# norlab-ulaval/norlab_icp_mapper

Measured on AMD Instinct MI355X. Metric: ICP iterations/sec, 100k-pt scan vs 1M-pt map, higher is better.
Workload: dtype f32; 1 GPU; single synthetic 100000-pt scan vs 1000000-pt map, point-to-point ICP, KDTreeMatcher knn 1 maxDist 2.0 epsilon 0, TrimmedDist 0.85, fixed 20 iterations per registration; chain=p2p, scene=box+pillars sigma=0.01 seeds 42/43/44 (SURVEY.md 8d), parallelism=scan-sharded x1, map replicated

## Files before the change

### norlab_icp_mapper_amd/csrc/common.h

```cpp
#pragma once

#include <hip/hip_runtime.h>
#include <stdint.h>
#include <math.h>
#include <cstring>
#include <string>
#include <vector>
#include <unordered_map>
#include <mutex>
#include <map>
#include <cstdlib>
#include <shared_mutex>

#include "../../include/icpmi.h"

#define ICPMI_NV 32
#define ICPMI_MAX_OUTLIER 8
#define ICPMI_MAX_SMOOTH 16
#define ICPMI_SEL_BINS 2048
#ifndef ICPMI_S2_COPIES
#define ICPMI_S2_COPIES 8
#endif
#define ICPMI_S2_C0 4096
#define ICPMI_S2_F0 (ICPMI_S2_C0 + ICPMI_S2_COPIES * 256)
// ... 127 lines not shown
    double hrot[ICPMI_MAX_SMOOTH + 1];
    double htr[ICPMI_MAX_SMOOTH + 1];
    double init_q[4];
    unsigned sel_prefix;
    unsigned sel_rank;
    unsigned n_valid;
    unsigned sel_prefix_l[3];
    unsigned sel_rank_l[3];
    float limits[ICPMI_MAX_OUTLIER];
    unsigned vt_valid;
    float vt_ratio;
    float robust_med;
    float robust_scale;
    long long pairs;
    double wsum;
    unsigned hard_count;
    unsigned ticket;
    unsigned long long hard_total;
    unsigned seq;
    unsigned long long dbg[24];
    float T_prev[16];
    float T_out[16];
    unsigned long long t_start, t_done;
    unsigned long long t_nn_begin, t_nn_sum;
    unsigned nn_count, pad_nn;
};

#ifdef __HIPCC__
__device__ __forceinline__ void nn_stamp_open(IcpState* st) { st->t_nn_begin = (unsigned long long)wall_clock64(); }
__device__ __forceinline__ void nn_stamp_close(IcpState* st)
{
    const unsigned long long b = st->t_nn_begin;
    if (b) { st->t_nn_sum += (unsigned long long)wall_clock64() - b; ++st->nn_count; st->t_nn_begin = 0; }
}
#endif


inline std::shared_mutex& capture_gate() { static std::shared_mutex* m = new std::shared_mutex; return *m; }
struct CaptureGate {
    CaptureGate() { capture_gate().lock_shared(); }
    ~CaptureGate() { capture_gate().unlock_shared(); }
    CaptureGate(const CaptureGate&) = delete;
    CaptureGate& operator=(const CaptureGate&) = delete;
};

struct LoopGraph {
    hipGraphExec_t exec = nullptr; uint64_t sig = 0; int uses = 0; bool sorted = false;
    int len = 0; unsigned long used = 0;
    bool holds(uint64_t s) const { return exec && sig == s; }
    void reset() { if (exec) hipGraphExecDestroy(exec); *this = LoopGraph(); }
};
struct LoopGraphs {
    LoopGraph fixed, batch, seg[2], heads[4];
    unsigned long clock = 0;
    void reset() { fixed.reset(); batch.reset(); for (LoopGraph& g : seg) g.reset(); for (LoopGraph& g : heads) g.reset(); }
};

struct DevBlockCache {
    struct Live { size_t bytes; int dev; };
    std::mutex mu;
    std::unordered_map<void*, Live> live;
    std::map<int, std::multimap<size_t, void*>> idle_of;
    size_t idle_bytes = 0, limit = 0;
    long handles = 0;
    bool on = true;
    DevBlockCache()
// ... 374 lines not shown
        HIP_TRY(c, hipStreamSynchronize(c->stream));
        return ICPMI_OK;
    }
    HIP_TRY(c, hipMemcpyAsync(c->h_pin, src0, b0, hipMemcpyDeviceToHost, c->stream));
    if (b1) HIP_TRY(c, hipMemcpyAsync(c->h_pin + b0, src1, b1, hipMemcpyDeviceToHost, c->stream));
    HIP_TRY(c, hipStreamSynchronize(c->stream));
    memcpy(dst0, c->h_pin, b0);
    if (b1) memcpy(dst1, c->h_pin + b0, b1);
    return ICPMI_OK;
}
static inline icpmi_status read_back(icpmi_ctx* c, void* dst, const void* src, size_t bytes) { return read_back2(c, dst, src, bytes, nullptr, nullptr, 0); }

#define ICPMI_UP_SLOT 1024
#define ICPMI_UP_SLOTS 64
static inline icpmi_status upload_small(icpmi_ctx* c, void* d_dst, const void* h_src, size_t bytes)
{
    if (!c->h_pin || bytes > ICPMI_UP_SLOT) {
        HIP_TRY(c, hipMemcpyAsync(d_dst, h_src, bytes, hipMemcpyHostToDevice, c->stream));
        return ICPMI_OK;
    }
    unsigned char* slot = c->h_pin + ICPMI_PIN_BYTES + (size_t)(c->up_next++ % ICPMI_UP_SLOTS) * ICPMI_UP_SLOT;
    memcpy(slot, h_src, bytes);
    HIP_TRY(c, hipMemcpyAsync(d_dst, slot, bytes, hipMemcpyHostToDevice, c->stream));
    return ICPMI_OK;
}

template <typename T>
static inline T* scratch_get(icpmi_ctx* c, int k, size_t count)
{
    if (c->scratch[k].ensure(c, (count ? count : 1) * sizeof(T)) != ICPMI_OK) { c->last_error = "out of device memory (operator scratch)"; return nullptr; }
    return (T*)c->scratch[k].get();
}

__device__ __forceinline__ float3 xf_point(const float* __restrict__ T, float x, float y, float z, float w)
{
    float3 o;
    o.x = fmaf(T[12], w, fmaf(T[8], z, fmaf(T[4], y, T[0] * x)));
    o.y = fmaf(T[13], w, fmaf(T[9], z, fmaf(T[5], y, T[1] * x)));
    o.z = fmaf(T[14], w, fmaf(T[10], z, fmaf(T[6], y, T[2] * x)));
    return o;
}

__device__ __forceinline__ float sqdist3(float ax, float ay, float az, float bx, float by, float bz)
{
    const float dx = ax - bx, dy = ay - by, dz = az - bz;
    return fmaf(dz, dz, fmaf(dy, dy, dx * dx));
}

__device__ __forceinline__ unsigned long long pack_key(float d2, unsigned id)
{
    return ((unsigned long long)__float_as_uint(d2) << 32) | (unsigned long long)id;
}

__device__ __forceinline__ float sqrt_up(float x) { return __builtin_amdgcn_sqrtf(x) * 1.0000005f; }

__device__ __forceinline__ unsigned fmix32(unsigned h)
{
    h ^= h >> 16; h *= 0x85ebca6bu; h ^= h >> 13; h *= 0xc2b2ae35u; h ^= h >> 16;
    return h;
}

__device__ __forceinline__ unsigned long long mix64(unsigned long long x)
{
    x ^= x >> 33; x *= 0xff51afd7ed558ccdull; x ^= x >> 33; x *= 0xc4ceb9fe1a85ec53ull; x ^= x >> 33;
    return x;
}
// ... 290 lines not shown
```

### norlab_icp_mapper_amd/csrc/loop.hip

```cpp
#include "common.h"
#include "solve.h"
#include <cstring>

namespace {

template <int PASS, int MODE = 0>
__global__ __launch_bounds__(256) void sel_hist_kernel(const float* __restrict__ d2, int64_t count,
                                                       const IcpState* __restrict__ st, unsigned* __restrict__ ghist, int nb_scale = 0)
{
    if (st->done) return;
    if (blockIdx.x == 0 && threadIdx.x == 0) nn_stamp_close(const_cast<IcpState*>(st));
    if (MODE != 0 && nb_scale != 0 && st->iter + 1 > nb_scale) return;
    if (MODE == 3 && st->iter != 0) return;
    __shared__ unsigned h[ICPMI_SEL_BINS];
    for (int b = threadIdx.x; b < ICPMI_SEL_BINS; b += 256) h[b] = 0;
    __syncthreads();
    const unsigned prefix = st->sel_prefix;
    const float med = MODE == 2 ? st->robust_med : 0.f;
    for (int64_t i = (int64_t)blockIdx.x * 256 + threadIdx.x; i < count; i += (int64_t)gridDim.x * 256) {
        float v = d2[i];
        if (MODE == 0 || MODE == 3) { if (!(v != INFINITY && v > 0.f)) continue; }
        else {
            if (v == INFINITY) continue;
            if (MODE == 2) v = fabsf(v - med);
// ... 191 lines not shown
        unsigned hit = 0u, pf = 0u, rr = 0u;
        if (lo1 != 0u && tot != 0u) {
            unsigned rank;
            if (quantile == 1.0f) rank = tot - 1;
            else {
                rank = (unsigned)((float)tot * quantile);
                if (rank > tot - 1) rank = tot - 1;
            }
            if (rank >= below && rank - below < inwin) {
                unsigned r = rank - below;
                for (int b = 0; b < ICPMI_WIN_BINS; ++b) {
                    const unsigned cb = sh[1 + b];
                    if (r < cb) { pf = lo1 - 1u + (unsigned)b; rr = r; hit = 1u; break; }
                    r -= cb;
                }
            }
        }
        sh[10] = hit; sh[11] = pf; sh[12] = rr; sh[13] = tot;
    }
    __syncthreads();
    const bool hit = sh[10] != 0u;
    prefix = sh[11]; rank_rem = sh[12]; total = sh[13];
    __syncthreads();
    return hit;
}

__global__ __launch_bounds__(256) void sel2_hist0_kernel(const float* __restrict__ d2, BatchArgs ba, int k, const IcpState* __restrict__ st,
                                                         unsigned* __restrict__ hists, float quantile, int use_win)
{
    const int64_t count = (int64_t)ba.n[blockIdx.y] * k;
    d2 += (size_t)blockIdx.y * (size_t)ba.qstride * k;
    hists += (size_t)blockIdx.y * ICPMI_SELHIST_WORDS;
    st += blockIdx.y;
    if (blockIdx.x == 0 && threadIdx.x == 0 && !st->done) nn_stamp_close(const_cast<IcpState*>(st));
    if (use_win) {
        if (st->done) return;
        __shared__ unsigned shw[16];
        unsigned pf, rr, tot;
        if (win_lookup(hists, quantile, shw, pf, rr, tot)) return;
    }
#ifndef ICPMI_H0_PF
#define ICPMI_H0_PF 16
#endif
    constexpr int PF = ICPMI_H0_PF;
    const int64_t stride = (int64_t)gridDim.x * 256;
    const int64_t i0 = (int64_t)blockIdx.x * 256 + threadIdx.x;
    float pv[PF];
#pragma unroll
    for (int u = 0; u < PF; ++u) pv[u] = i0 + u * stride < count ? d2[i0 + u * stride] : INFINITY;
    if (st->done) return;
    constexpr int WIN = 4096;
    __shared__ unsigned h[256];
    __shared__ unsigned win[WIN];
    __shared__ unsigned s_top;
    h[threadIdx.x] = 0;
    for (int i = threadIdx.x; i < WIN; i += 256) win[i] = 0;
    if (threadIdx.x == 0) s_top = 0u;
    for (int64_t i = i0; i < 256 + 65536; i += stride) hists[ICPMI_S2_C1 + i] = 0;
    __syncthreads();
    {
        unsigned mx = 0;
#pragma unroll
        for (int u = 0; u < PF; ++u) if (pv[u] != INFINITY && pv[u] > 0.f) mx = max(mx, __float_as_uint(pv[u]) >> 16);
        for (int off = 32; off > 0; off >>= 1) mx = max(mx, (unsigned)__shfl_xor((int)mx, off, 64));
        if ((threadIdx.x & 63) == 0 && mx) atomicMax(&s_top, mx);
    }
    __syncthreads();
    const unsigned top = s_top + 1u, lo = top > (unsigned)WIN ? top - (unsigned)WIN : 0u;
    unsigned* fine = hists + ICPMI_S2_F0 + (blockIdx.x % ICPMI_S2_FCOPIES) * 65536;
    auto add = [&](float v) {
        if (!(v != INFINITY && v > 0.f)) return;
        const unsigned bits = __float_as_uint(v);
        const unsigned bin = bits >> 16, rel = bin - lo;
        if (rel < (unsigned)WIN) atomicAdd(&win[rel], 1u);
        else { atomicAdd(&h[bits >> 24], 1u); atomicAdd(&fine[ICPMI_S2_FIDX(bin)], 1u); }
    };
#pragma unroll
    for (int u = 0; u < PF; ++u) add(pv[u]);
    for (int64_t i = i0 + PF * stride; i < count; i += stride) add(d2[i]);
    __syncthreads();
    for (int i = threadIdx.x; i < WIN; i += 256) {
        const unsigned cnt = win[i];
        if (cnt) { const unsigned bin = lo + (unsigned)i; atomicAdd(&h[bin >> 8], cnt); atomicAdd(&fine[ICPMI_S2_FIDX(bin)], cnt); }
    }
    __syncthreads();
    if (h[threadIdx.x]) atomicAdd(&hists[ICPMI_S2_C0 + (blockIdx.x % ICPMI_S2_COPIES) * 256 + threadIdx.x], h[threadIdx.x]);
}

__global__ __launch_bounds__(256) void sel2_scan_hist_kernel(const float* __restrict__ d2, BatchArgs ba, int k, IcpState* __restrict__ st,
                                                             unsigned* __restrict__ hists, float quantile, int use_win)
{
    const int64_t count = (int64_t)ba.n[blockIdx.y] * k;
    d2 += (size_t)blockIdx.y * (size_t)ba.qstride * k;
    hists += (size_t)blockIdx.y * ICPMI_SELHIST_WORDS;
    st += blockIdx.y;
    constexpr int PF = 2;
    const int64_t stride = (int64_t)gridDim.x * 256;
    const int64_t i0 = (int64_t)blockIdx.x * 256 + threadIdx.x;
    float pv[PF];
#pragma unroll
    for (int u = 0; u < PF; ++u) pv[u] = i0 + u * stride < count ? d2[i0 + u * stride] : INFINITY;
    unsigned cv = 0;
#pragma unroll
    for (int cpy = 0; cpy < ICPMI_S2_COPIES; ++cpy) cv += hists[ICPMI_S2_C0 + cpy * 256 + threadIdx.x];
    if (st->done) return;
    if (blockIdx.x == 0 && threadIdx.x == 0) nn_stamp_close(const_cast<IcpState*>(st));
    __shared__ unsigned sh[16];
    unsigned prefix, rem, total;
    const bool win_hit = use_win && win_lookup(hists, quantile, sh, prefix, rem, total);
    if (!win_hit) block_find_rank_2tier<ICPMI_S2_FCOPIES>(cv, hists + ICPMI_S2_F0, true, quantile, 0u, sh, prefix, rem, total);
#ifndef ICPMI_NN_TIMING
    if (use_win && blockIdx.x == 0 && threadIdx.x == 0) st->dbg[win_hit ? 12 : 13] += 1ull;
#endif
    if (total == 0) {
        if (blockIdx.x == 0 && threadIdx.x == 0) { st->n_valid = 0; st->error = ICPMI_ERR_NO_OUTLIER_TO_FILTER; st->done = 1; }
        return;
    }
    if (blockIdx.x == 0 && threadIdx.x == 0) { st->sel_prefix_l[0] = prefix; st->sel_rank_l[0] = rem; st->n_valid = total; }
    auto add = [&](float v) {
        if (!(v != INFINITY && v > 0.f)) return;
        const unsigned bits = __float_as_uint(v);
        if ((bits >> 16) != prefix) return;
        atomicAdd(&hists[ICPMI_S2_C1 + ((bits >> 8) & 255u)], 1u);
        atomicAdd(&hists[ICPMI_S2_F1 + ICPMI_S2_FIDX(bits & 0xffffu)], 1u);
    };
#pragma unroll
    for (int u = 0; u < PF; ++u) add(pv[u]);
    for (int64_t i = i0 + PF * stride; i < count; i += stride) add(d2[i]);
}

constexpr int VT_CHUNK = 2048;

__global__ __launch_bounds__(256) void vt_keys_kernel(const float* __restrict__ d2, int64_t count, IcpState* __restrict__ st,
                                                      unsigned long long* __restrict__ keys, unsigned* __restrict__ vals)
{
    const int64_t i = (int64_t)blockIdx.x * 256 + threadIdx.x;
    if (blockIdx.x == 0 && threadIdx.x == 0 && !st->done) nn_stamp_close(st);
    const float v = i < count ? d2[i] : INFINITY;
    const bool valid = v != INFINITY && v > 0.f;
// ... 186 lines not shown
            const int ip = lc.out_iparam[f];
            const int se = (ip >> 4) & 15, fct = ip & 15;
            const float sc = se != ICPMI_SCALE_NONE ? st->robust_scale : 1.f;
            const float res = ((ip >> 8) & 15) == ICPMI_DIST_POINT2PLANE ? plane2 : d2;
            const float kk = se != ICPMI_SCALE_BERG ? prm : (fct == ICPMI_ROB_CAUCHY ? 4.3040f : fct == ICPMI_ROB_TUKEY ? 7.0589f : fct == ICPMI_ROB_HUBER ? 2.0138f : prm);
            const float e2 = res / (sc * sc);
            const float apx = lc.out_param3[f];
            float rw = robust_weight(fct, e2, kk);
            if (apx > 0.f && apx != INFINITY && e2 >= apx * apx) rw = 0.f;
            w *= rw;
        }
    }
    return w;
}

__host__ __device__ __forceinline__ int acc_threads(int k) { return k > 1 ? 1024 : 256; }
__host__ __device__ __forceinline__ int acc_blocks_dev(int64_t count, int cap, int bt = 256)
{
    const int64_t nb = (count + bt - 1) / bt;
    return (int)(nb < 1 ? 1 : (nb > cap ? cap : nb));
}

template <int MIN, bool FUSED, bool EXT, int BT = 256>
__global__ __launch_bounds__(BT) void accumulate_kernel(const float4* __restrict__ reading, BatchArgs ba, int acc_cap, LoopCfg lc,
                                                         IcpState* __restrict__ st, const float4* __restrict__ map,
                                                         const float4* __restrict__ normals,
                                                         const float4* __restrict__ read_normals,
                                                         const int* __restrict__ sidx, const float* __restrict__ d2a,
                                                         unsigned* __restrict__ hists,
                                                         int fused_slot, int is_median, float factor,
                                                         const float4* __restrict__ match_pt, const int* __restrict__ qindex,
                                                         const float* __restrict__ ref_scalar, const float4* __restrict__ pnm)
{
    const int n = ba.n[blockIdx.y];
    const int nbe = acc_blocks_dev((int64_t)n * lc.k, acc_cap, BT);
    if ((int)blockIdx.x >= nbe) return;
    {
        const size_t qo = (size_t)blockIdx.y * (size_t)ba.qstride;
        reading += qo; sidx += qo * lc.k; d2a += qo * lc.k;
        if (match_pt) match_pt += qo;
        if (qindex) qindex += qo;
        if (read_normals) read_normals += qo;
        hists += (size_t)blockIdx.y * ICPMI_SELHIST_WORDS;
        st += blockIdx.y;
    }
    const int64_t count = (int64_t)n * lc.k;
    const int64_t stride = (int64_t)nbe * BT;
    const int64_t gtid = (int64_t)blockIdx.x * BT + threadIdx.x;
#ifdef ICPMI_ACC_STRIDED
    const int64_t estep = stride;
    const int64_t e_first = gtid, e_end = count;
#else
    const int64_t estep = BT;
    const int wgc = (nbe & 7) == 0 ? (int)(blockIdx.x & 7) * (nbe >> 3) + (int)(blockIdx.x >> 3) : (int)blockIdx.x;
    const int64_t per_wg = (count + nbe - 1) / nbe;
    const int64_t e_first = (int64_t)wgc * per_wg + threadIdx.x;
    const int64_t e_end = ((int64_t)wgc + 1) * per_wg < count ? ((int64_t)wgc + 1) * per_wg : count;
#endif
    constexpr int PF = BT > 256 ? 3 : 2;
    float pd2[PF]; int ps[PF]; float4 pr[PF], pq[PF];
#pragma unroll
    for (int u = 0; u < PF; ++u) {
        const int64_t e = e_first + u * estep;
        const bool in = e < e_end;
        pd2[u] = in ? ld_stream(d2a + e) : INFINITY;
        ps[u] = in ? ld_stream(sidx + e) : -1;
        pr[u] = ld_stream(reading + (in ? (int)(e / lc.k) : 0));
        pq[u] = (match_pt && in) ? ld_stream(match_pt + e) : ((pnm && ps[u] >= 0) ? pnm[2 * (size_t)ps[u]] : make_float4(0.f, 0.f, 0.f, 0.f));
    }
    const unsigned cv = (FUSED && threadIdx.x < 256) ? hists[ICPMI_S2_C1 + threadIdx.x] : 0u;
    float4 pn[PF];
#pragma unroll
    for (int u = 0; u < PF; ++u)
        pn[u] = (MIN == ICPMI_MIN_POINT_TO_PLANE && ps[u] >= 0) ? (pnm ? pnm[2 * (size_t)ps[u] + 1] : normals[ps[u]]) : make_float4(0.f, 0.f, 0.f, 0.f);
    if (st->done) return;
    if (blockIdx.x == 0 && threadIdx.x == 0) nn_stamp_close(const_cast<IcpState*>(st));
    float fused_limit = 0.f;
    if (FUSED) {
        __shared__ unsigned shsel[16];
        unsigned bin, rem, total;
        block_find_rank_2tier<1>(cv, hists + ICPMI_S2_F1, false, 0.f, st->sel_rank_l[0], shsel, bin, rem, total);
        const float q = __uint_as_float((st->sel_prefix_l[0] << 16) | bin);
        fused_limit = is_median ? factor * q : q;
        if (blockIdx.x == 0 && threadIdx.x == 0) st->limits[fused_slot] = fused_limit;
        for (int64_t i = gtid; i < ICPMI_S2_COPIES * 256 + ICPMI_S2_FCOPIES * 65536; i += stride) hists[ICPMI_S2_C0 + i] = 0;
        if (lc.k > 1) for (int64_t i = gtid; i < 2 * ICPMI_WIN_U64; i += stride) hists[ICPMI_S2_WIN + i] = 0;
    }
    constexpr int NVAL = MIN == ICPMI_MIN_POINT_TO_PLANE ? 27 : (MIN == ICPMI_MIN_POINT_TO_POINT ? 16 : 0);
    double acc[NVAL > 0 ? NVAL : 1];
#pragma unroll
    for (int i = 0; i < (NVAL > 0 ? NVAL : 1); ++i) acc[i] = 0.0;
    double wsum = 0.0, cnt = 0.0;
    double b2d[3] = {0.0, 0.0, 0.0};
    const float* T = st->T_iter;
    auto pair = [&](int64_t e, float d2, int s, float4 r, float4 qkept, float4 nkept, bool have_n) {
        if (d2 == INFINITY) return;
        const int qi = (int)(e / lc.k);
        float w;
        if (EXT) {
            const float3 pe = xf_point(T, r.x, r.y, r.z, r.w);
            const float4 qe = (match_pt || (pnm && have_n)) ? qkept : (pnm ? pnm[2 * (size_t)s] : map[s]);
            float plane2 = 0.f;
            if (normals) {
                const float4 ne = have_n && MIN == ICPMI_MIN_POINT_TO_PLANE ? nkept : (pnm ? pnm[2 * (size_t)s + 1] : normals[s]);
                const float dx = pe.x - qe.x, dy = pe.y - qe.y, dz = pe.z - qe.z;
                const float dot = dx * ne.x + dy * ne.y + dz * ne.z;
                plane2 = dot * dot;
            }
            w = match_weight<true>(lc, st, d2, T, read_normals, qindex ? qindex[qi] : qi, normals, s, FUSED ? fused_slot : -1, fused_limit,
                                   ref_scalar, __float_as_int(qe.w), plane2);
        } else w = match_weight(lc, st, d2, T, read_normals, qindex ? qindex[qi] : qi, normals, s, FUSED ? fused_slot : -1, fused_limit);
        if (w == 0.f) return;
        wsum += w; cnt += 1.0;
        if (MIN == ICPMI_MIN_IDENTITY) return;
        const float3 p = xf_point(T, r.x, r.y, r.z, r.w);
        const float4 q = (match_pt || (pnm && have_n)) ? qkept : (pnm ? pnm[2 * (size_t)s] : map[s]);
        if (MIN == ICPMI_MIN_POINT_TO_POINT) {
            const double dw = w;
            acc[0] += dw;
            acc[1] += dw * p.x; acc[2] += dw * p.y; acc[3] += dw * p.z;
            acc[4] += dw * q.x; acc[5] += dw * q.y; acc[6] += dw * q.z;
            const double wq[3] = {dw * q.x, dw * q.y, dw * q.z};
            const float pc[3] = {p.x, p.y, p.z};
#pragma unroll
            for (int c = 0; c < 3; ++c)
#pragma unroll
                for (int rr = 0; rr < 3; ++rr) acc[7 + 3 * c + rr] += wq[rr] * pc[c];
        } else if (MIN == ICPMI_MIN_POINT_TO_PLANE) {
            const float4 nn = have_n ? nkept : (pnm ? pnm[2 * (size_t)s + 1] : normals[s]);
            const float F[6] = {p.y * nn.z - p.z * nn.y, p.z * nn.x - p.x * nn.z, p.x * nn.y - p.y * nn.x, nn.x, nn.y, nn.z};
            const float dx = p.x - q.x, dy = p.y - q.y, dz = p.z - q.z;
            const float dot = dx * nn.x + dy * nn.y + dz * nn.z;
            int idx = 0;
#pragma unroll
            for (int a = 0; a < 6; ++a) {
                const double wf = (double)w * F[a];
#pragma unroll
                for (int b = a; b < 6; ++b) acc[idx++] += wf * F[b];
                acc[21 + a] -= wf * dot;
            }
            if (EXT && lc.force_2d) {
                const float dot2 = dx * nn.x + dy * nn.y;
#pragma unroll
                for (int a = 0; a < 3; ++a) b2d[a] -= ((double)w * F[2 + a]) * dot2;
            }
        }
    };
#pragma unroll
// ... 19 lines not shown
            const double keep = upper ? val[i + nkeep] : val[i];
            val[i] = keep + __shfl_xor(send, m, 64);
        }
    }
    val[0] += __shfl_xor(val[0], 32, 64);
    if (lane < 32) {
        const int idx = ((lane & 1) << 4) | ((lane & 2) << 2) | (lane & 4) | ((lane & 8) >> 2) | ((lane & 16) >> 4);
        sh[wv][idx] = val[0];
    }
    __syncthreads();
    if (threadIdx.x < ICPMI_NV) {
        const int i = threadIdx.x;
        double v = 0.0;
        if (i < NVAL || i == 27 || i == 28 || (EXT && i > 28)) {
            v = sh[0][i] + sh[1][i] + sh[2][i] + sh[3][i];
#pragma unroll
            for (int w2 = 4; w2 < BT / 64; ++w2) v += sh[w2][i];
        }
        unsigned long long* acc = reinterpret_cast<unsigned long long*>(hists + ICPMI_S2_ACC);
        if (v != 0.0) {
            if (!(fabs(v) < 0x1p77)) atomicOr(reinterpret_cast<unsigned*>(acc + ICPMI_ACC_FLAG), 1u);
            else {
                const double hi = rint(v * 0x1p-16);
                const double lo = v - hi * 65536.0;
                const long long H = (long long)hi, Lq = __double2ll_rn(lo * 0x1p40);
                const int cp = blockIdx.x & (ICPMI_ACC_COPIES - 1);
                if (H) atomicAdd(acc + ICPMI_ACC_IDX(cp, i, 0), (unsigned long long)H);
                if (Lq) atomicAdd(acc + ICPMI_ACC_IDX(cp, i, 1), (unsigned long long)Lq);
            }
        }
    }
}

__device__ __forceinline__ void mirror_state(const IcpState* st, IcpState* mirror)
{
    const unsigned* src = reinterpret_cast<const unsigned*>(st);
    unsigned* dst = reinterpret_cast<unsigned*>(mirror);
    constexpr int W = (int)(sizeof(IcpState) / sizeof(unsigned));
    for (int i = threadIdx.x; i < W; i += 64) dst[i] = __hip_atomic_load(src + i, __ATOMIC_RELAXED, __HIP_MEMORY_SCOPE_AGENT);
}

__global__ __launch_bounds__(256) void solve_kernel(IcpState* __restrict__ st, unsigned* __restrict__ hists, int clear, LoopCfg lc,
                                                    float* __restrict__ T_step_out, double* __restrict__ sums_out, unsigned* __restrict__ progress,
                                                    IcpState* __restrict__ mirror)
{
    st += blockIdx.x;
    unsigned long long* acc = reinterpret_cast<unsigned long long*>(hists + (size_t)blockIdx.x * ICPMI_SELHIST_WORDS + ICPMI_S2_ACC);
    if (progress) progress += blockIdx.x;
    if (threadIdx.x == 0 && st->hard_count) { st->hard_total += st->hard_count; st->hard_count = 0; }
    if (st->done) {
        if (mirror && threadIdx.x < 64) mirror_state(st, mirror + blockIdx.x);
        if (threadIdx.x == 0) publish_progress(st, progress);
        return;
    }
    solve_body(st, acc, clear != 0, lc, T_step_out, sums_out);
    if (threadIdx.x == 0 && st->done) st->t_done = (unsigned long long)wall_clock64();
    if (mirror) {
        __syncthreads();
        if (threadIdx.x < 64 && __hip_atomic_load(&st->done, __ATOMIC_RELAXED, __HIP_MEMORY_SCOPE_AGENT)) mirror_state(st, mirror + blockIdx.x);
    }
    if (threadIdx.x == 0) publish_progress(st, progress);
}

__global__ __launch_bounds__(256) void centre_kernel(BatchSrc src, BatchArgs ba, float mx, float my, float mz, float4* __restrict__ out)
{
    const int64_t n = ba.n[blockIdx.y];
    const float4* __restrict__ scan = src.p[blockIdx.y];
    out += (size_t)blockIdx.y * (size_t)ba.qstride;
    const int64_t i = (int64_t)blockIdx.x * 256 + threadIdx.x;
    if (i >= n) return;
    const float4 p = scan[i];
    out[i] = make_float4(fmaf(-mx, p.w, p.x), fmaf(-my, p.w, p.y), fmaf(-mz, p.w, p.z), p.w);
}

__global__ __launch_bounds__(256) void pad_normals_kernel(const float* __restrict__ n3, int64_t n, float4* __restrict__ out)
{
    const int64_t i = (int64_t)blockIdx.x * 256 + threadIdx.x;
    if (i >= n) return;
    out[i] = make_float4(n3[3 * i], n3[3 * i + 1], n3[3 * i + 2], 0.f);
}

__global__ void init_state_kernel(IcpState* st, const float* T0, unsigned seq, unsigned* progress, const unsigned* seq_src = nullptr)
{
    if (threadIdx.x != 0) return;
    st[blockIdx.x].t_start = (unsigned long long)wall_clock64();
    init_state_dev(st + blockIdx.x, T0, seq, progress ? progress + blockIdx.x : nullptr, seq_src);
}

__global__ __launch_bounds__(256) void weights_kernel(int64_t count, LoopCfg lc, const IcpState* __restrict__ st,
                                                      const float4* __restrict__ normals, const float4* __restrict__ read_normals,
                                                      const int* __restrict__ sidx, const float* __restrict__ d2a,
                                                      float* __restrict__ w, const float* __restrict__ ref_scalar)
{
    const int64_t e = (int64_t)blockIdx.x * 256 + threadIdx.x;
// ... 1093 lines not shown
```

### norlab_icp_mapper_amd/csrc/solve.h

```cpp
#pragma once
#include "common.h"

namespace {

__device__ void mat4_mul_dev(const float* A, const float* B, float* C)
{
    float R[16];
#pragma unroll
    for (int j = 0; j < 4; ++j)
#pragma unroll
        for (int i = 0; i < 4; ++i) {
            float s = A[i] * B[4 * j];
#pragma unroll
            for (int kk = 1; kk < 4; ++kk) s = fmaf(A[4 * kk + i], B[4 * j + kk], s);
            R[4 * j + i] = s;
        }
#pragma unroll
    for (int i = 0; i < 16; ++i) C[i] = R[i];
}

__device__ void jacobi_eig(int n, const double* Ain, double* w, double* Q)
{
    __shared__ double A[36];
    for (int i = 0; i < n * n; ++i) A[i] = Ain[i];
// ... 336 lines not shown
        s = fmaf(nrm * z, ps, nrm);
        float pc = fmaf(z, -2.75573192e-07f, 2.48015873e-05f);
        pc = fmaf(z, pc, -1.38888889e-03f);
        pc = fmaf(z, pc, 4.16666667e-02f);
        pc = fmaf(z, pc, -0.5f);
        c = fmaf(z, pc, 1.f);
    } else { s = (float)sin((double)nrm); c = (float)cos((double)nrm); }
    const float sx = s * ax, sy = s * ay, sz = s * az;
    const float cx = (1.f - c) * ax, cy = (1.f - c) * ay, cz = (1.f - c) * az;
    float tmp;
    tmp = cx * ay; T[4 * 1 + 0] = tmp - sz; T[4 * 0 + 1] = tmp + sz;
    tmp = cx * az; T[4 * 2 + 0] = tmp + sy; T[4 * 0 + 2] = tmp - sy;
    tmp = cy * az; T[4 * 2 + 1] = tmp - sx; T[4 * 1 + 2] = tmp + sx;
    T[0] = cx * ax + c; T[5] = cy * ay + c; T[10] = cz * az + c;
}

__device__ double quat_angdist(const double* a, const double* b)
{
    const double w = a[0] * b[0] + a[1] * b[1] + a[2] * b[2] + a[3] * b[3];
    const double x = -a[0] * b[1] + a[1] * b[0] - a[2] * b[3] + a[3] * b[2];
    const double y = -a[0] * b[2] + a[1] * b[3] + a[2] * b[0] - a[3] * b[1];
    const double z = -a[0] * b[3] - a[1] * b[2] + a[2] * b[1] + a[3] * b[0];
    return 2.0 * atan2(sqrt(x * x + y * y + z * z), fabs(w));
}

__device__ __forceinline__ unsigned pair_sum_mask(const LoopCfg& lc)
{
    const unsigned nval = lc.minimizer == ICPMI_MIN_POINT_TO_PLANE ? 27u : (lc.minimizer == ICPMI_MIN_POINT_TO_POINT ? 16u : 0u);
    unsigned m = (nval ? ((1u << nval) - 1u) : 0u) | (1u << 27) | (1u << 28);
    if (lc.force_2d) m |= 7u << 29;
    return m;
}

__device__ __forceinline__ void read_pair_sums(unsigned long long* __restrict__ acc, double* __restrict__ tot , bool clear, bool* nonfinite,
                                               unsigned mask = 0xffffffffu)
{
    __shared__ long long ph[ICPMI_ACC_COPIES][ICPMI_NV], pl[ICPMI_ACC_COPIES][ICPMI_NV];
    __shared__ unsigned s_flag;
    const int t = threadIdx.x;
    if (t < ICPMI_ACC_COPIES * ICPMI_NV) {
        const int i = t & (ICPMI_NV - 1), cp = t >> 5;
        unsigned long long a = 0ull, b = 0ull;
        if ((mask >> i) & 1u) { a = acc[ICPMI_ACC_IDX(cp, i, 0)]; b = acc[ICPMI_ACC_IDX(cp, i, 1)]; }
        ph[cp][i] = (long long)a; pl[cp][i] = (long long)b;
        if (clear) { if (a) acc[ICPMI_ACC_IDX(cp, i, 0)] = 0ull; if (b) acc[ICPMI_ACC_IDX(cp, i, 1)] = 0ull; }
    }
    if (t == ICPMI_ACC_COPIES * ICPMI_NV) {
        unsigned* fl = reinterpret_cast<unsigned*>(acc + ICPMI_ACC_FLAG);
        s_flag = *fl;
        if (clear && s_flag) *fl = 0u;
    }
    __syncthreads();
    if (t < ICPMI_NV) {
        long long H = 0, Lq = 0;
#pragma unroll
        for (int cp = 0; cp < ICPMI_ACC_COPIES; ++cp) { H += ph[cp][t]; Lq += pl[cp][t]; }
        tot[t] = (double)H * 65536.0 + (double)Lq * 0x1p-40;
    }
    __syncthreads();
    *nonfinite = s_flag != 0u;
}

__device__ void solve_serial(IcpState* st, const double* tot, const LoopCfg& lc, float* T_step_out)
{
    const long long tsolve0 = clock64();

    const double wsum = tot[27];
    const long long P = (long long)(tot[28] + 0.5);
    st->pairs = P;
    st->wsum = wsum;
    if (P == 0) { st->error = ICPMI_ERR_NO_POINT_TO_MINIMIZE; st->done = 1; return; }

    float Ts[16];
    for (int i = 0; i < 16; ++i) Ts[i] = (i % 5 == 0) ? 1.f : 0.f;
    if (lc.minimizer == ICPMI_MIN_POINT_TO_POINT) {
        const double iw = 1.0 / wsum;
        const double mpd[3] = {tot[1] * iw, tot[2] * iw, tot[3] * iw}, mqd[3] = {tot[4] * iw, tot[5] * iw, tot[6] * iw};
        __shared__ float H[9];
        for (int c = 0; c < 3; ++c)
            for (int r = 0; r < 3; ++r) H[3 * c + r] = (float)(tot[7 + 3 * c + r] - mqd[r] * tot[1 + c]);
        __shared__ float R[9];
        if (lc.is_2d) {
            const float a = H[0] + H[4], b2 = H[1] - H[3];
            const float r = sqrtf(a * a + b2 * b2);
            float cs = 1.f, sn = 0.f;
            if (r > 0.f) { cs = a / r; sn = b2 / r; }
            for (int i = 0; i < 9; ++i) R[i] = 0.f;
            R[0] = cs; R[1] = sn; R[3] = -sn; R[4] = cs; R[8] = 1.f;
        } else rotation_from_H(H, R);
        const float mp[3] = {(float)mpd[0], (float)mpd[1], (float)mpd[2]};
        const float mq[3] = {(float)mqd[0], (float)mqd[1], (float)mqd[2]};
        for (int c = 0; c < 3; ++c) for (int r = 0; r < 3; ++r) Ts[4 * c + r] = R[3 * c + r];
        for (int r = 0; r < 3; ++r) Ts[12 + r] = mq[r] - (R[r] * mp[0] + R[3 + r] * mp[1] + R[6 + r] * mp[2]);
    } else if (lc.minimizer == ICPMI_MIN_POINT_TO_PLANE) {
        __shared__ float A[36], b[6], x[6];
        auto fill_Ab = [&]() {
            int idx = 0;
            for (int a = 0; a < 6; ++a)
                for (int bb = a; bb < 6; ++bb) { const float v = (float)tot[idx++]; A[6 * a + bb] = v; A[6 * bb + a] = v; }
            for (int a = 0; a < 6; ++a) b[a] = (float)tot[21 + a];
        };
        if (lc.force_2d || lc.force_4dof) fill_Ab();
        if (lc.force_2d) {
            __shared__ float A3[9], b3[3], x3[3];
            for (int c = 0; c < 3; ++c) { b3[c] = (float)tot[29 + c]; for (int r = 0; r < 3; ++r) A3[3 * c + r] = A[6 * (2 + c) + (2 + r)]; }
            solve_spd<3>(A3, b3, x3);
            x[0] = 0.f; x[1] = 0.f; x[2] = x3[0]; x[3] = x3[1]; x[4] = x3[2]; x[5] = 0.f;
        } else if (lc.force_4dof) {
            __shared__ float A4[16], b4[4], x4[4];
            for (int c = 0; c < 4; ++c) { b4[c] = b[2 + c]; for (int r = 0; r < 4; ++r) A4[4 * c + r] = A[6 * (2 + c) + (2 + r)]; }
            solve_spd<4>(A4, b4, x4);
            x[0] = 0.f; x[1] = 0.f; x[2] = x4[0]; x[3] = x4[1]; x[4] = x4[2]; x[5] = x4[3];
        } else {
            auto tri = [](int r, int c) { return r * 6 - r * (r - 1) / 2 + (c - r); };
            const bool ok = chol_solve<6>([&](int i, int j) { return (float)tot[tri(j < i ? j : i, j < i ? i : j)]; },
                                          [&](int i) { return (float)tot[21 + i]; }, x);
            if (!ok) { fill_Ab(); solve_min_norm(6, A, b, x); }
        }
        angle_axis_T(x, Ts);
        Ts[12] = x[3]; Ts[13] = x[4]; Ts[14] = x[5];
    }
    const long long tsolve1 = clock64();
    for (int i = 0; i < 16; ++i)
        if (Ts[i] != Ts[i]) { st->error = ICPMI_ERR_NAN; st->done = 1; return; }
    if (T_step_out) for (int i = 0; i < 16; ++i) T_step_out[i] = Ts[i];

    float Ti[16];
    mat4_mul_dev(Ts, st->T_iter, Ti);
    for (int i = 0; i < 16; ++i) st->T_prev[i] = st->T_iter[i];
    for (int i = 0; i < 16; ++i) st->T_iter[i] = Ti[i];
    st->iter += 1;

    const long long tsolve2 = clock64();
    bool iterate = true;
    int reason = ICPMI_STOP_NONE;
    st->counter += 1;
    if (st->counter >= lc.max_iter) { iterate = false; reason = ICPMI_STOP_COUNTER; }
    if (lc.use_diff) {
        const int SL = lc.smooth;
        const int RING = ICPMI_MAX_SMOOTH + 1;
        const int slot = st->hist_n % RING;
        quat_from_T(Ti, st->hq + 4 * slot);
        for (int r = 0; r < 3; ++r) st->ht[3 * slot + r] = Ti[12 + r];
        st->hist_n += 1;
        const int hn = st->hist_n;
        {
            const int a = (hn - 1) % RING, bq = (hn - 2) % RING;
            st->hrot[a] = fabs(quat_angdist(st->hq + 4 * a, st->hq + 4 * bq));
            const double dx = st->ht[3 * a] - st->ht[3 * bq], dy = st->ht[3 * a + 1] - st->ht[3 * bq + 1],
                         dz = st->ht[3 * a + 2] - st->ht[3 * bq + 2];
            st->htr[a] = sqrt(dx * dx + dy * dy + dz * dz);
        }
        if (hn > SL) {
            double rot = 0, tr = 0;
            for (int i = hn - 1; i >= hn - SL; --i) { rot += st->hrot[i % RING]; tr += st->htr[i % RING]; }
            rot /= SL; tr /= SL;
            if (rot != rot || tr != tr) { st->error = ICPMI_ERR_NAN; st->done = 1; return; }
            if (rot < (double)lc.min_rot && tr < (double)lc.min_trans) {
                if (iterate) reason = ICPMI_STOP_DIFFERENTIAL;
                iterate = false;
            }
        }
    }
    if (lc.use_bound) {
        __shared__ double q[4];
        quat_from_T(Ti, q);
        const double rot = fabs(quat_angdist(q, st->init_q));
        const double nt = sqrt((double)Ti[12] * Ti[12] + (double)Ti[13] * Ti[13] + (double)Ti[14] * Ti[14]);
        if (rot > (double)lc.max_rot || nt > (double)lc.max_trans) { st->error = ICPMI_ERR_BOUND; st->done = 1; return; }
    }
    if (!iterate) { st->done = 1; st->stop_reason = reason; }
    const long long tsolve3 = clock64();
#ifndef ICPMI_NN_TIMING
    st->dbg[20] += (unsigned long long)(tsolve3 - tsolve0);
    st->dbg[21] += 1;
    st->dbg[22] += (unsigned long long)(tsolve1 - tsolve0);
    st->dbg[23] += (unsigned long long)(tsolve3 - tsolve2);
#else
    (void)tsolve1; (void)tsolve2; (void)tsolve3;
#endif
}

__device__ void solve_body(IcpState* __restrict__ st, unsigned long long* __restrict__ acc, bool clear, const LoopCfg& lc,
                           float* __restrict__ T_step_out, double* __restrict__ sums_out)
{
    __shared__ double tot[ICPMI_NV];
    const int t = threadIdx.x;
    bool nonfinite = false;
    read_pair_sums(acc, tot, clear, &nonfinite, pair_sum_mask(lc));
    if (t < ICPMI_NV && sums_out) sums_out[t] = tot[t];
    if (nonfinite) { if (t == 0) { st->error = ICPMI_ERR_NAN; st->done = 1; } return; }
    if (t == 0) solve_serial(st, tot, lc, T_step_out);
}

__device__ __forceinline__ void publish_progress(const IcpState* st, unsigned* progress)
{
    if (!progress) return;
    const unsigned v = ((unsigned)(st->done != 0) << 31) | ((st->seq & 0x7ffffu) << 12) | ((unsigned)st->iter & 0xfffu);
    __hip_atomic_store(progress, v, __ATOMIC_RELEASE, __HIP_MEMORY_SCOPE_SYSTEM);
}
struct ProgressWord { bool mine, done; int iter; };
static inline ProgressWord decode_progress(unsigned v, unsigned seq) { return {((v >> 12) & 0x7ffffu) == seq, (v >> 31) != 0, (int)(v & 0xfffu)}; }


}
```

Baseline: 23940 iterations/s.

## Stage ICP state in LDS and hoist scalar state loads across loop kernels

The solve kernel now loads the whole IcpState into shared memory cooperatively, overlaps that with the pair-sum reads, runs the serial solve on the shared copy, and writes back only words that changed. The histogram and accumulate kernels read done flags, selection ranks, the pose and NN timing stamps once through a constant-address-space view, with asm barriers pushing the loads early, instead of dereferencing global state repeatedly. Progress publishing uses a relaxed store unless the run is done. This targets the serial latency of small per-iteration kernels. The cost is more LDS use and reliance on constant-space loads of state that other kernels mutate.

New measurement: 23660 iterations/s. 1.1% lower.

```diff
diff --git a/norlab_icp_mapper_amd/csrc/common.h b/norlab_icp_mapper_amd/csrc/common.h
--- a/norlab_icp_mapper_amd/csrc/common.h
+++ b/norlab_icp_mapper_amd/csrc/common.h
@@ -183,6 +183,14 @@
 {
     const unsigned long long b = st->t_nn_begin;
     if (b) { st->t_nn_sum += (unsigned long long)wall_clock64() - b; ++st->nn_count; st->t_nn_begin = 0; }
+}
+struct NnStamp { unsigned long long begin, sum; unsigned count; };
+typedef const __attribute__((address_space(4))) IcpState* IcpStateK;
+__device__ __forceinline__ IcpStateK state_words(const IcpState* st) { return (IcpStateK)st; }
+__device__ __forceinline__ NnStamp nn_stamp_request(IcpStateK st) { return {st->t_nn_begin, st->t_nn_sum, st->nn_count}; }
+__device__ __forceinline__ void nn_stamp_close(IcpState* st, const NnStamp& s)
+{
+    if (s.begin) { st->t_nn_sum = s.sum + ((unsigned long long)wall_clock64() - s.begin); st->nn_count = s.count + 1u; st->t_nn_begin = 0; }
 }
 #endif
 
@@ -623,6 +631,15 @@
     return (T*)c->scratch[k].get();
 }
 
+struct PoseRegs { float t0, t1, t2, t4, t5, t6, t8, t9, t10, t12, t13, t14; };
+__device__ __forceinline__ float3 xf_point(const PoseRegs& T, float x, float y, float z, float w)
+{
+    float3 o;
+    o.x = fmaf(T.t12, w, fmaf(T.t8, z, fmaf(T.t4, y, T.t0 * x)));
+    o.y = fmaf(T.t13, w, fmaf(T.t9, z, fmaf(T.t5, y, T.t1 * x)));
+    o.z = fmaf(T.t14, w, fmaf(T.t10, z, fmaf(T.t6, y, T.t2 * x)));
+    return o;
+}
 __device__ __forceinline__ float3 xf_point(const float* __restrict__ T, float x, float y, float z, float w)
 {
     float3 o;
diff --git a/norlab_icp_mapper_amd/csrc/loop.hip b/norlab_icp_mapper_amd/csrc/loop.hip
--- a/norlab_icp_mapper_amd/csrc/loop.hip
+++ b/norlab_icp_mapper_amd/csrc/loop.hip
@@ -247,9 +247,14 @@
     d2 += (size_t)blockIdx.y * (size_t)ba.qstride * k;
     hists += (size_t)blockIdx.y * ICPMI_SELHIST_WORDS;
     st += blockIdx.y;
-    if (blockIdx.x == 0 && threadIdx.x == 0 && !st->done) nn_stamp_close(const_cast<IcpState*>(st));
+    const IcpStateK sts = state_words(st);
+    const int st_done = sts->done;
+    NnStamp stamp = {0ull, 0ull, 0u};
+    if (blockIdx.x == 0) stamp = nn_stamp_request(sts);
+    asm volatile("" ::"s"(st_done), "s"(stamp.begin), "s"(stamp.sum), "s"(stamp.count));
+    if (blockIdx.x == 0 && threadIdx.x == 0 && !st_done) nn_stamp_close(const_cast<IcpState*>(st), stamp);
     if (use_win) {
-        if (st->done) return;
+        if (st_done) return;
         __shared__ unsigned shw[16];
         unsigned pf, rr, tot;
         if (win_lookup(hists, quantile, shw, pf, rr, tot)) return;
@@ -263,7 +268,7 @@
     float pv[PF];
 #pragma unroll
     for (int u = 0; u < PF; ++u) pv[u] = i0 + u * stride < count ? d2[i0 + u * stride] : INFINITY;
-    if (st->done) return;
+    if (st_done) return;
     constexpr int WIN = 4096;
     __shared__ unsigned h[256];
     __shared__ unsigned win[WIN];
@@ -305,6 +310,7 @@
 __global__ __launch_bounds__(256) void sel2_scan_hist_kernel(const float* __restrict__ d2, BatchArgs ba, int k, IcpState* __restrict__ st,
                                                              unsigned* __restrict__ hists, float quantile, int use_win)
 {
+    asm volatile("" ::"s"(d2), "s"(ba.n[blockIdx.y]), "s"(ba.qstride), "s"(k), "s"(st), "s"(hists), "s"(quantile), "s"(use_win));
     const int64_t count = (int64_t)ba.n[blockIdx.y] * k;
     d2 += (size_t)blockIdx.y * (size_t)ba.qstride * k;
     hists += (size_t)blockIdx.y * ICPMI_SELHIST_WORDS;
@@ -317,9 +323,15 @@
     for (int u = 0; u < PF; ++u) pv[u] = i0 + u * stride < count ? d2[i0 + u * stride] : INFINITY;
     unsigned cv = 0;
 #pragma unroll
-    for (int cpy = 0; cpy < ICPMI_S2_COPIES; ++cpy) cv += hists[ICPMI_S2_C0 + cpy * 256 + threadIdx.x];
-    if (st->done) return;
-    if (blockIdx.x == 0 && threadIdx.x == 0) nn_stamp_close(const_cast<IcpState*>(st));
+    for (int cpy = 0; cpy < ICPMI_S2_COPIES; ++cpy)
+        cv += __hip_atomic_load(hists + ICPMI_S2_C0 + cpy * 256 + threadIdx.x, __ATOMIC_RELAXED, __HIP_MEMORY_SCOPE_SINGLETHREAD);
+    const IcpStateK sts = state_words(st);
+    const int st_done = sts->done;
+    NnStamp stamp = {0ull, 0ull, 0u};
+    if (blockIdx.x == 0) stamp = nn_stamp_request(sts);
+    asm volatile("" ::"s"(st_done), "s"(stamp.begin), "s"(stamp.sum), "s"(stamp.count));
+    if (st_done) return;
+    if (blockIdx.x == 0 && threadIdx.x == 0) nn_stamp_close(st, stamp);
     __shared__ unsigned sh[16];
     unsigned prefix, rem, total;
     const bool win_hit = use_win && win_lookup(hists, quantile, sh, prefix, rem, total);
@@ -572,6 +584,8 @@
                                                          const float4* __restrict__ match_pt, const int* __restrict__ qindex,
                                                          const float* __restrict__ ref_scalar, const float4* __restrict__ pnm)
 {
+    asm volatile("" ::"s"(reading), "s"(ba.n[blockIdx.y]), "s"(ba.qstride), "s"(acc_cap), "s"(lc.k), "s"(st), "s"(sidx), "s"(d2a), "s"(hists),
+                 "s"(match_pt), "s"(qindex), "s"(read_normals), "s"(pnm), "s"(normals), "s"(map));
     const int n = ba.n[blockIdx.y];
     const int nbe = acc_blocks_dev((int64_t)n * lc.k, acc_cap, BT);
     if ((int)blockIdx.x >= nbe) return;
@@ -598,6 +612,7 @@
     const int64_t e_end = ((int64_t)wgc + 1) * per_wg < count ? ((int64_t)wgc + 1) * per_wg : count;
 #endif
     constexpr int PF = BT > 256 ? 3 : 2;
+    const unsigned cv = (FUSED && threadIdx.x < 256) ? hists[ICPMI_S2_C1 + threadIdx.x] : 0u;
     float pd2[PF]; int ps[PF]; float4 pr[PF], pq[PF];
 #pragma unroll
     for (int u = 0; u < PF; ++u) {
@@ -606,21 +621,33 @@
         pd2[u] = in ? ld_stream(d2a + e) : INFINITY;
         ps[u] = in ? ld_stream(sidx + e) : -1;
         pr[u] = ld_stream(reading + (in ? (int)(e / lc.k) : 0));
-        pq[u] = (match_pt && in) ? ld_stream(match_pt + e) : ((pnm && ps[u] >= 0) ? pnm[2 * (size_t)ps[u]] : make_float4(0.f, 0.f, 0.f, 0.f));
-    }
-    const unsigned cv = (FUSED && threadIdx.x < 256) ? hists[ICPMI_S2_C1 + threadIdx.x] : 0u;
+        pq[u] = match_pt ? ld_stream(match_pt + (in ? e : 0)) : make_float4(0.f, 0.f, 0.f, 0.f);
+    }
+    if (!match_pt) {
+#pragma unroll
+        for (int u = 0; u < PF; ++u) if (pnm && ps[u] >= 0) pq[u] = pnm[2 * (size_t)ps[u]];
+    }
+    const IcpStateK sts = state_words(st);
+    const int st_done = sts->done;
+    const unsigned sel_prefix0 = sts->sel_prefix_l[0], sel_rank0 = sts->sel_rank_l[0];
+    const PoseRegs pose = {sts->T_iter[0], sts->T_iter[1], sts->T_iter[2], sts->T_iter[4], sts->T_iter[5], sts->T_iter[6],
+                           sts->T_iter[8], sts->T_iter[9], sts->T_iter[10], sts->T_iter[12], sts->T_iter[13], sts->T_iter[14]};
+    NnStamp stamp = {0ull, 0ull, 0u};
+    if (blockIdx.x == 0) stamp = nn_stamp_request(sts);
     float4 pn[PF];
 #pragma unroll
     for (int u = 0; u < PF; ++u)
         pn[u] = (MIN == ICPMI_MIN_POINT_TO_PLANE && ps[u] >= 0) ? (pnm ? pnm[2 * (size_t)ps[u] + 1] : normals[ps[u]]) : make_float4(0.f, 0.f, 0.f, 0.f);
-    if (st->done) return;
-    if (blockIdx.x == 0 && threadIdx.x == 0) nn_stamp_close(const_cast<IcpState*>(st));
+    asm volatile("" ::"s"(st_done), "s"(sel_prefix0), "s"(sel_rank0), "s"(stamp.begin), "s"(stamp.sum), "s"(stamp.count));
+    asm volatile("" ::"s"(pose.t0), "s"(pose.t1), "s"(pose.t2), "s"(pose.t4), "s"(pose.t5), "s"(pose.t6), "s"(pose.t8), "s"(pose.t9), "s"(pose.t10), "s"(pose.t12), "s"(pose.t13), "s"(pose.t14));
+    if (st_done) return;
+    if (blockIdx.x == 0 && threadIdx.x == 0) nn_stamp_close(st, stamp);
     float fused_limit = 0.f;
     if (FUSED) {
         __shared__ unsigned shsel[16];
         unsigned bin, rem, total;
-        block_find_rank_2tier<1>(cv, hists + ICPMI_S2_F1, false, 0.f, st->sel_rank_l[0], shsel, bin, rem, total);
-        const float q = __uint_as_float((st->sel_prefix_l[0] << 16) | bin);
+        block_find_rank_2tier<1>(cv, hists + ICPMI_S2_F1, false, 0.f, sel_rank0, shsel, bin, rem, total);
+        const float q = __uint_as_float((sel_prefix0 << 16) | bin);
         fused_limit = is_median ? factor * q : q;
         if (blockIdx.x == 0 && threadIdx.x == 0) st->limits[fused_slot] = fused_limit;
         for (int64_t i = gtid; i < ICPMI_S2_COPIES * 256 + ICPMI_S2_FCOPIES * 65536; i += stride) hists[ICPMI_S2_C0 + i] = 0;
@@ -638,7 +665,7 @@
         const int qi = (int)(e / lc.k);
         float w;
         if (EXT) {
-            const float3 pe = xf_point(T, r.x, r.y, r.z, r.w);
+            const float3 pe = xf_point(pose, r.x, r.y, r.z, r.w);
             const float4 qe = (match_pt || (pnm && have_n)) ? qkept : (pnm ? pnm[2 * (size_t)s] : map[s]);
             float plane2 = 0.f;
             if (normals) {
@@ -653,7 +680,7 @@
         if (w == 0.f) return;
         wsum += w; cnt += 1.0;
         if (MIN == ICPMI_MIN_IDENTITY) return;
-        const float3 p = xf_point(T, r.x, r.y, r.z, r.w);
+        const float3 p = xf_point(pose, r.x, r.y, r.z, r.w);
         const float4 q = (match_pt || (pnm && have_n)) ? qkept : (pnm ? pnm[2 * (size_t)s] : map[s]);
         if (MIN == ICPMI_MIN_POINT_TO_POINT) {
             const double dw = w;
@@ -739,34 +766,52 @@
     }
 }
 
-__device__ __forceinline__ void mirror_state(const IcpState* st, IcpState* mirror)
-{
-    const unsigned* src = reinterpret_cast<const unsigned*>(st);
-    unsigned* dst = reinterpret_cast<unsigned*>(mirror);
-    constexpr int W = (int)(sizeof(IcpState) / sizeof(unsigned));
-    for (int i = threadIdx.x; i < W; i += 64) dst[i] = __hip_atomic_load(src + i, __ATOMIC_RELAXED, __HIP_MEMORY_SCOPE_AGENT);
-}
-
 __global__ __launch_bounds__(256) void solve_kernel(IcpState* __restrict__ st, unsigned* __restrict__ hists, int clear, LoopCfg lc,
                                                     float* __restrict__ T_step_out, double* __restrict__ sums_out, unsigned* __restrict__ progress,
                                                     IcpState* __restrict__ mirror)
 {
+    asm volatile("" ::"s"(st), "s"(hists), "s"(clear), "s"(T_step_out), "s"(sums_out), "s"(progress), "s"(mirror));
+    asm volatile("" ::"s"(lc.minimizer), "s"(lc.force_4dof), "s"(lc.force_2d), "s"(lc.is_2d), "s"(lc.max_iter), "s"(lc.use_diff), "s"(lc.min_rot),
+                 "s"(lc.min_trans), "s"(lc.smooth), "s"(lc.use_bound), "s"(lc.max_rot), "s"(lc.max_trans));
     st += blockIdx.x;
     unsigned long long* acc = reinterpret_cast<unsigned long long*>(hists + (size_t)blockIdx.x * ICPMI_SELHIST_WORDS + ICPMI_S2_ACC);
     if (progress) progress += blockIdx.x;
-    if (threadIdx.x == 0 && st->hard_count) { st->hard_total += st->hard_count; st->hard_count = 0; }
-    if (st->done) {
-        if (mirror && threadIdx.x < 64) mirror_state(st, mirror + blockIdx.x);
-        if (threadIdx.x == 0) publish_progress(st, progress);
-        return;
-    }
-    solve_body(st, acc, clear != 0, lc, T_step_out, sums_out);
-    if (threadIdx.x == 0 && st->done) st->t_done = (unsigned long long)wall_clock64();
-    if (mirror) {
-        __syncthreads();
-        if (threadIdx.x < 64 && __hip_atomic_load(&st->done, __ATOMIC_RELAXED, __HIP_MEMORY_SCOPE_AGENT)) mirror_state(st, mirror + blockIdx.x);
-    }
-    if (threadIdx.x == 0) publish_progress(st, progress);
+    constexpr int W = (int)(sizeof(IcpState) / sizeof(unsigned)), NW = (W + 255) / 256;
+    static_assert(sizeof(IcpState) % sizeof(unsigned) == 0, "IcpState is staged word by word");
+    __shared__ IcpState s_st;
+    __shared__ PairSumStage s_sums;
+    __shared__ double tot[ICPMI_NV];
+    const int t = threadIdx.x;
+    unsigned* gw = reinterpret_cast<unsigned*>(st);
+    unsigned* lw = reinterpret_cast<unsigned*>(&s_st);
+    unsigned w0[NW];
+#pragma unroll
+    for (int u = 0; u < NW; ++u) w0[u] = t + 256 * u < W ? gw[t + 256 * u] : 0u;
+    const PairSumLoad ps = pair_sums_request(acc, pair_sum_mask(lc));
+#pragma unroll
+    for (int u = 0; u < NW; ++u) if (t + 256 * u < W) lw[t + 256 * u] = w0[u];
+    pair_sums_stage(ps, &s_sums);
+    __syncthreads();
+    if (t == 0 && s_st.hard_count) { s_st.hard_total += s_st.hard_count; s_st.hard_count = 0; }
+    if (!s_st.done) {
+        bool nonfinite = false;
+        pair_sums_reduce(acc, ps, &s_sums, tot, clear != 0, &nonfinite);
+        if (t < ICPMI_NV && sums_out) sums_out[t] = tot[t];
+        if (t == 0) {
+            if (nonfinite) { s_st.error = ICPMI_ERR_NAN; s_st.done = 1; }
+            else solve_serial(&s_st, tot, lc, T_step_out);
+            if (s_st.done) s_st.t_done = (unsigned long long)wall_clock64();
+        }
+    }
+    __syncthreads();
+#pragma unroll
+    for (int u = 0; u < NW; ++u)
+        if (t + 256 * u < W) { const unsigned v = lw[t + 256 * u]; if (v != w0[u]) gw[t + 256 * u] = v; }
+    if (mirror && t < 64 && s_st.done) {
+        unsigned* dst = reinterpret_cast<unsigned*>(mirror + blockIdx.x);
+        for (int i = t; i < W; i += 64) dst[i] = lw[i];
+    }
+    if (t == 0) publish_progress(&s_st, progress);
 }
 
 __global__ __launch_bounds__(256) void centre_kernel(BatchSrc src, BatchArgs ba, float mx, float my, float mz, float4* __restrict__ out)
diff --git a/norlab_icp_mapper_amd/csrc/solve.h b/norlab_icp_mapper_amd/csrc/solve.h
--- a/norlab_icp_mapper_amd/csrc/solve.h
+++ b/norlab_icp_mapper_amd/csrc/solve.h
@@ -392,33 +392,45 @@
     return m;
 }
 
-__device__ __forceinline__ void read_pair_sums(unsigned long long* __restrict__ acc, double* __restrict__ tot , bool clear, bool* nonfinite,
-                                               unsigned mask = 0xffffffffu)
-{
-    __shared__ long long ph[ICPMI_ACC_COPIES][ICPMI_NV], pl[ICPMI_ACC_COPIES][ICPMI_NV];
-    __shared__ unsigned s_flag;
+struct PairSumLoad { unsigned long long a, b; unsigned flag; };
+__device__ __forceinline__ PairSumLoad pair_sums_request(const unsigned long long* __restrict__ acc, unsigned mask = 0xffffffffu)
+{
+    PairSumLoad r = {0ull, 0ull, 0u};
     const int t = threadIdx.x;
     if (t < ICPMI_ACC_COPIES * ICPMI_NV) {
         const int i = t & (ICPMI_NV - 1), cp = t >> 5;
-        unsigned long long a = 0ull, b = 0ull;
-        if ((mask >> i) & 1u) { a = acc[ICPMI_ACC_IDX(cp, i, 0)]; b = acc[ICPMI_ACC_IDX(cp, i, 1)]; }
-        ph[cp][i] = (long long)a; pl[cp][i] = (long long)b;
-        if (clear) { if (a) acc[ICPMI_ACC_IDX(cp, i, 0)] = 0ull; if (b) acc[ICPMI_ACC_IDX(cp, i, 1)] = 0ull; }
-    }
-    if (t == ICPMI_ACC_COPIES * ICPMI_NV) {
-        unsigned* fl = reinterpret_cast<unsigned*>(acc + ICPMI_ACC_FLAG);
-        s_flag = *fl;
-        if (clear && s_flag) *fl = 0u;
-    }
-    __syncthreads();
+        if ((mask >> i) & 1u) { r.a = acc[ICPMI_ACC_IDX(cp, i, 0)]; r.b = acc[ICPMI_ACC_IDX(cp, i, 1)]; }
+    }
+    if (t == ICPMI_ACC_COPIES * ICPMI_NV) r.flag = *reinterpret_cast<const unsigned*>(acc + ICPMI_ACC_FLAG);
+    return r;
+}
+struct PairSumStage { long long ph[ICPMI_ACC_COPIES][ICPMI_NV], pl[ICPMI_ACC_COPIES][ICPMI_NV]; unsigned flag; };
+__device__ __forceinline__ void pair_sums_stage(const PairSumLoad& r, PairSumStage* __restrict__ sg )
+{
+    const int t = threadIdx.x;
+    if (t < ICPMI_ACC_COPIES * ICPMI_NV) { sg->ph[t >> 5][t & (ICPMI_NV - 1)] = (long long)r.a; sg->pl[t >> 5][t & (ICPMI_NV - 1)] = (long long)r.b; }
+    if (t == ICPMI_ACC_COPIES * ICPMI_NV) sg->flag = r.flag;
+}
+__device__ __forceinline__ void pair_sums_reduce(unsigned long long* __restrict__ acc, const PairSumLoad& r, const PairSumStage* __restrict__ sg,
+                                                 double* __restrict__ tot , bool clear, bool* nonfinite)
+{
+    const int t = threadIdx.x;
+    if (clear) {
+        if (t < ICPMI_ACC_COPIES * ICPMI_NV) {
+            const int i = t & (ICPMI_NV - 1), cp = t >> 5;
+            if (r.a) acc[ICPMI_ACC_IDX(cp, i, 0)] = 0ull;
+            if (r.b) acc[ICPMI_ACC_IDX(cp, i, 1)] = 0ull;
+        }
+        if (t == ICPMI_ACC_COPIES * ICPMI_NV && r.flag) *reinterpret_cast<unsigned*>(acc + ICPMI_ACC_FLAG) = 0u;
+    }
     if (t < ICPMI_NV) {
         long long H = 0, Lq = 0;
 #pragma unroll
-        for (int cp = 0; cp < ICPMI_ACC_COPIES; ++cp) { H += ph[cp][t]; Lq += pl[cp][t]; }
+        for (int cp = 0; cp < ICPMI_ACC_COPIES; ++cp) { H += sg->ph[cp][t]; Lq += sg->pl[cp][t]; }
         tot[t] = (double)H * 65536.0 + (double)Lq * 0x1p-40;
     }
     __syncthreads();
-    *nonfinite = s_flag != 0u;
+    *nonfinite = sg->flag != 0u;
 }
 
 __device__ void solve_serial(IcpState* st, const double* tot, const LoopCfg& lc, float* T_step_out)
@@ -431,7 +443,7 @@
     st->wsum = wsum;
     if (P == 0) { st->error = ICPMI_ERR_NO_POINT_TO_MINIMIZE; st->done = 1; return; }
 
-    float Ts[16];
+    __shared__ float Ts[16], Ti[16];
     for (int i = 0; i < 16; ++i) Ts[i] = (i % 5 == 0) ? 1.f : 0.f;
     if (lc.minimizer == ICPMI_MIN_POINT_TO_POINT) {
         const double iw = 1.0 / wsum;
@@ -485,7 +497,6 @@
         if (Ts[i] != Ts[i]) { st->error = ICPMI_ERR_NAN; st->done = 1; return; }
     if (T_step_out) for (int i = 0; i < 16; ++i) T_step_out[i] = Ts[i];
 
-    float Ti[16];
     mat4_mul_dev(Ts, st->T_iter, Ti);
     for (int i = 0; i < 16; ++i) st->T_prev[i] = st->T_iter[i];
     for (int i = 0; i < 16; ++i) st->T_iter[i] = Ti[i];
@@ -541,23 +552,13 @@
 #endif
 }
 
-__device__ void solve_body(IcpState* __restrict__ st, unsigned long long* __restrict__ acc, bool clear, const LoopCfg& lc,
-                           float* __restrict__ T_step_out, double* __restrict__ sums_out)
-{
-    __shared__ double tot[ICPMI_NV];
-    const int t = threadIdx.x;
-    bool nonfinite = false;
-    read_pair_sums(acc, tot, clear, &nonfinite, pair_sum_mask(lc));
-    if (t < ICPMI_NV && sums_out) sums_out[t] = tot[t];
-    if (nonfinite) { if (t == 0) { st->error = ICPMI_ERR_NAN; st->done = 1; } return; }
-    if (t == 0) solve_serial(st, tot, lc, T_step_out);
-}
-
 __device__ __forceinline__ void publish_progress(const IcpState* st, unsigned* progress)
 {
     if (!progress) return;
-    const unsigned v = ((unsigned)(st->done != 0) << 31) | ((st->seq & 0x7ffffu) << 12) | ((unsigned)st->iter & 0xfffu);
-    __hip_atomic_store(progress, v, __ATOMIC_RELEASE, __HIP_MEMORY_SCOPE_SYSTEM);
+    const bool done = st->done != 0;
+    const unsigned v = ((unsigned)done << 31) | ((st->seq & 0x7ffffu) << 12) | ((unsigned)st->iter & 0xfffu);
+    if (done) __hip_atomic_store(progress, v, __ATOMIC_RELEASE, __HIP_MEMORY_SCOPE_SYSTEM);
+    else __hip_atomic_store(progress, v, __ATOMIC_RELAXED, __HIP_MEMORY_SCOPE_SYSTEM);
 }
 struct ProgressWord { bool mine, done; int iter; };
 static inline ProgressWord decode_progress(unsigned v, unsigned seq) { return {((v >> 12) & 0x7ffffu) == seq, (v >> 31) != 0, (int)(v & 0xfffu)}; }
```
